# snayfach/MIDAS

Measured on AMD Instinct MI355X. Metric: genomic sites/sec pileup+allele-count, higher is better.
Workload: dtype u8/u32 integer tallies (fp64 only in the two keep_read ratio tests)

## Files before the change

midas_amd/csrc/device_common.h:

```cpp
#pragma once
#include "kernels.h"

namespace midas {
namespace dev {

enum : uint32_t { OP_M = 0, OP_I = 1, OP_D = 2, OP_N = 3, OP_S = 4, OP_H = 5, OP_P = 6, OP_EQ = 7, OP_X = 8 };

enum : uint32_t {
  E_NO_SEQ = 1,
  E_NO_NM = 2,
  E_ZERO_ALIGN = 3,
  E_NO_QUAL = 4,
  E_CIGAR_OVERRUN = 5,
};

typedef uint32_t u32x4_a8 __attribute__((ext_vector_type(4), aligned(8)));
typedef uint32_t u32x4_a4 __attribute__((ext_vector_type(4), aligned(4)));
typedef uint32_t u32x4_a1 __attribute__((ext_vector_type(4), aligned(1)));

__device__ __forceinline__ bool consumes_both(uint32_t op) { return op == OP_M || op == OP_EQ || op == OP_X; }

__device__ __forceinline__ int rec_pos(const uint4& r) { return (int)r.x; }
__device__ __forceinline__ uint32_t rec_off8(const uint4& r) { return r.y; }
__device__ __forceinline__ int rec_l(const uint4& r) { return (int)(r.z & 0x7FFu); }
__device__ __forceinline__ int seg_read_l(const uint4& r) { return (int)((r.z >> 16) & 0x3FFu); }
__device__ __forceinline__ int seg_align_len(const uint4& r) { return (int)((((r.z >> 26) & 0xFu) << 6) | ((r.w >> 10) & 0x3Fu)); }
__device__ __forceinline__ int seg_nm(const uint4& r) { return (int)(r.w & 0x3FFu); }
__device__ __forceinline__ bool seg_first(const uint4& r) { return ((r.z >> 30) & 1u) != 0u; }
__device__ __forceinline__ int rec_qmean(const uint4& r) { return (int)(((r.z >> 11) & 31u) | ((r.w >> 23) & 0xE0u)); }
__device__ __forceinline__ int rec_n(const uint4& r) { return (int)(r.z >> 16); }
__device__ __forceinline__ uint32_t rec_nm(const uint4& r) { return r.w & 0xFFFFu; }
__device__ __forceinline__ int rec_mapq(const uint4& r) { return (int)((r.w >> 16) & 0xFFu); }
__device__ __forceinline__ uint32_t rec_flags(const uint4& r) { return r.w >> 24; }


}
}
```

midas_amd/csrc/pileup_direct.hip:

```cpp
#include "direct_common.h"
#include "pileup_common.h"

#include <type_traits>

namespace midas {

using namespace dev;
using namespace pile;
using namespace direct;

namespace {

#ifdef MIDAS_ISA_MARKS
#define MIDAS_MARK(name) asm volatile("; MARK " name)
#else
#define MIDAS_MARK(name) do { } while (0)
#endif

__device__ __forceinline__ void lds_barrier() { asm volatile("s_waitcnt lgkmcnt(0)\n\ts_barrier" ::: "memory"); }

template <int OFF, int NB>
__device__ __forceinline__ void tally_group(uint32_t b0, uint32_t b1, uint32_t thr, uint32_t abase, uint32_t one) {
  static_assert(NB == 8 || NB == 6, "a group holds 8 bases, or 6 at the end of a 30-base lane");
  const uint32_t c0 = (b0 << 2) & 0x0C0C0C0Cu, c1 = (b1 << 2) & 0x0C0C0C0Cu;
  uint32_t t0, t1, t2, t3, t4, t5, t6, t7;
  unsigned long long m0, m1, m2, m3, m4, m5, m6, m7, save;
  if (NB == 8) {
    asm volatile(
        "v_or_b32_sdwa %[t0], %[ab], %[c0] dst_sel:DWORD dst_unused:UNUSED_PAD src0_sel:DWORD src1_sel:BYTE_0\n\t"
        "v_or_b32_sdwa %[t1], %[ab], %[c0] dst_sel:DWORD dst_unused:UNUSED_PAD src0_sel:DWORD src1_sel:BYTE_1\n\t"
        "v_or_b32_sdwa %[t2], %[ab], %[c0] dst_sel:DWORD dst_unused:UNUSED_PAD src0_sel:DWORD src1_sel:BYTE_2\n\t"
        "v_or_b32_sdwa %[t3], %[ab], %[c0] dst_sel:DWORD dst_unused:UNUSED_PAD src0_sel:DWORD src1_sel:BYTE_3\n\t"
        "v_or_b32_sdwa %[t4], %[ab], %[c1] dst_sel:DWORD dst_unused:UNUSED_PAD src0_sel:DWORD src1_sel:BYTE_0\n\t"
        "v_or_b32_sdwa %[t5], %[ab], %[c1] dst_sel:DWORD dst_unused:UNUSED_PAD src0_sel:DWORD src1_sel:BYTE_1\n\t"
        "v_or_b32_sdwa %[t6], %[ab], %[c1] dst_sel:DWORD dst_unused:UNUSED_PAD src0_sel:DWORD src1_sel:BYTE_2\n\t"
        "v_or_b32_sdwa %[t7], %[ab], %[c1] dst_sel:DWORD dst_unused:UNUSED_PAD src0_sel:DWORD src1_sel:BYTE_3\n\t"
        "v_cmp_ge_u32_sdwa %[m0], %[b0], %[th] src0_sel:BYTE_0 src1_sel:DWORD\n\t"
        "v_cmp_ge_u32_sdwa %[m1], %[b0], %[th] src0_sel:BYTE_1 src1_sel:DWORD\n\t"
        "v_cmp_ge_u32_sdwa %[m2], %[b0], %[th] src0_sel:BYTE_2 src1_sel:DWORD\n\t"
        "v_cmp_ge_u32_sdwa %[m3], %[b0], %[th] src0_sel:BYTE_3 src1_sel:DWORD\n\t"
        "v_cmp_ge_u32_sdwa %[m4], %[b1], %[th] src0_sel:BYTE_0 src1_sel:DWORD\n\t"
        "v_cmp_ge_u32_sdwa %[m5], %[b1], %[th] src0_sel:BYTE_1 src1_sel:DWORD\n\t"
        "v_cmp_ge_u32_sdwa %[m6], %[b1], %[th] src0_sel:BYTE_2 src1_sel:DWORD\n\t"
        "v_cmp_ge_u32_sdwa %[m7], %[b1], %[th] src0_sel:BYTE_3 src1_sel:DWORD\n\t"
        "s_mov_b64 %[sv], exec\n\t"
        "s_mov_b64 exec, %[m0]\n\t"
        "ds_add_u32 %[t0], %[one] offset:%[off]\n\t"
        "s_mov_b64 exec, %[m1]\n\t"
        "ds_add_u32 %[t1], %[one] offset:%[off]+16\n\t"
        "s_mov_b64 exec, %[m2]\n\t"
        "ds_add_u32 %[t2], %[one] offset:%[off]+32\n\t"
        "s_mov_b64 exec, %[m3]\n\t"
        "ds_add_u32 %[t3], %[one] offset:%[off]+48\n\t"
        "s_mov_b64 exec, %[m4]\n\t"
        "ds_add_u32 %[t4], %[one] offset:%[off]+64\n\t"
        "s_mov_b64 exec, %[m5]\n\t"
        "ds_add_u32 %[t5], %[one] offset:%[off]+80\n\t"
        "s_mov_b64 exec, %[m6]\n\t"
        "ds_add_u32 %[t6], %[one] offset:%[off]+96\n\t"
        "s_mov_b64 exec, %[m7]\n\t"
        "ds_add_u32 %[t7], %[one] offset:%[off]+112\n\t"
        "s_mov_b64 exec, %[sv]"
        : [t0] "=&v"(t0), [t1] "=&v"(t1), [t2] "=&v"(t2), [t3] "=&v"(t3), [t4] "=&v"(t4), [t5] "=&v"(t5), [t6] "=&v"(t6),
          [t7] "=&v"(t7), [m0] "=&s"(m0), [m1] "=&s"(m1), [m2] "=&s"(m2), [m3] "=&s"(m3), [m4] "=&s"(m4), [m5] "=&s"(m5),
          [m6] "=&s"(m6), [m7] "=&s"(m7), [sv] "=&s"(save)
        : [b0] "v"(b0), [b1] "v"(b1), [th] "v"(thr), [c0] "v"(c0), [c1] "v"(c1), [ab] "v"(abase), [one] "v"(one), [off] "n"(OFF)
        : "memory");
  } else {
    asm volatile(
        "v_or_b32_sdwa %[t0], %[ab], %[c0] dst_sel:DWORD dst_unused:UNUSED_PAD src0_sel:DWORD src1_sel:BYTE_0\n\t"
        "v_or_b32_sdwa %[t1], %[ab], %[c0] dst_sel:DWORD dst_unused:UNUSED_PAD src0_sel:DWORD src1_sel:BYTE_1\n\t"
        "v_or_b32_sdwa %[t2], %[ab], %[c0] dst_sel:DWORD dst_unused:UNUSED_PAD src0_sel:DWORD src1_sel:BYTE_2\n\t"
        "v_or_b32_sdwa %[t3], %[ab], %[c0] dst_sel:DWORD dst_unused:UNUSED_PAD src0_sel:DWORD src1_sel:BYTE_3\n\t"
        "v_or_b32_sdwa %[t4], %[ab], %[c1] dst_sel:DWORD dst_unused:UNUSED_PAD src0_sel:DWORD src1_sel:BYTE_0\n\t"
        "v_or_b32_sdwa %[t5], %[ab], %[c1] dst_sel:DWORD dst_unused:UNUSED_PAD src0_sel:DWORD src1_sel:BYTE_1\n\t"
        "v_cmp_ge_u32_sdwa %[m0], %[b0], %[th] src0_sel:BYTE_0 src1_sel:DWORD\n\t"
        "v_cmp_ge_u32_sdwa %[m1], %[b0], %[th] src0_sel:BYTE_1 src1_sel:DWORD\n\t"
        "v_cmp_ge_u32_sdwa %[m2], %[b0], %[th] src0_sel:BYTE_2 src1_sel:DWORD\n\t"
        "v_cmp_ge_u32_sdwa %[m3], %[b0], %[th] src0_sel:BYTE_3 src1_sel:DWORD\n\t"
        "v_cmp_ge_u32_sdwa %[m4], %[b1], %[th] src0_sel:BYTE_0 src1_sel:DWORD\n\t"
        "v_cmp_ge_u32_sdwa %[m5], %[b1], %[th] src0_sel:BYTE_1 src1_sel:DWORD\n\t"
        "s_mov_b64 %[sv], exec\n\t"
        "s_mov_b64 exec, %[m0]\n\t"
        "ds_add_u32 %[t0], %[one] offset:%[off]\n\t"
        "s_mov_b64 exec, %[m1]\n\t"
        "ds_add_u32 %[t1], %[one] offset:%[off]+16\n\t"
        "s_mov_b64 exec, %[m2]\n\t"
        "ds_add_u32 %[t2], %[one] offset:%[off]+32\n\t"
        "s_mov_b64 exec, %[m3]\n\t"
        "ds_add_u32 %[t3], %[one] offset:%[off]+48\n\t"
        "s_mov_b64 exec, %[m4]\n\t"
        "ds_add_u32 %[t4], %[one] offset:%[off]+64\n\t"
        "s_mov_b64 exec, %[m5]\n\t"
        "ds_add_u32 %[t5], %[one] offset:%[off]+80\n\t"
        "s_mov_b64 exec, %[sv]"
        : [t0] "=&v"(t0), [t1] "=&v"(t1), [t2] "=&v"(t2), [t3] "=&v"(t3), [t4] "=&v"(t4), [t5] "=&v"(t5), [m0] "=&s"(m0),
          [m1] "=&s"(m1), [m2] "=&s"(m2), [m3] "=&s"(m3), [m4] "=&s"(m4), [m5] "=&s"(m5), [sv] "=&s"(save)
        : [b0] "v"(b0), [b1] "v"(b1), [th] "v"(thr), [c0] "v"(c0), [c1] "v"(c1), [ab] "v"(abase), [one] "v"(one), [off] "n"(OFF)
        : "memory");
  }
}

struct Stream { int rb, n0, total; };

#ifndef MIDAS_DIRECT_BLOCK
#define MIDAS_DIRECT_BLOCK 256
#endif
constexpr int kDirectBlock = MIDAS_DIRECT_BLOCK;
static_assert(kDirectBlock % 64 == 0 && kDirectBlock >= 128 && kDirectBlock <= 1024, "whole wavefronts");
constexpr int kDirectWavesPerSimd = (kWorkgroupsPerCU * kDirectBlock / 64 + 3) / 4;


template <int LB, bool BQ0, int OV = kDirectOverhang>
__global__ __launch_bounds__(kDirectBlock, kDirectWavesPerSimd) void pileup_direct_kernel(DirectParams p) {
  constexpr int TILE = kTileSites;
  constexpr int NWAVES = kDirectBlock / 64;
  constexpr int OUT_IT = (TILE + kDirectBlock - 1) / kDirectBlock;
  static_assert(OV <= TILE, "the overhang is moved by the write-out's first rounds");
  __shared__ __attribute__((aligned(16))) uint32_t lds[4 * (TILE + OV)];
  __shared__ __attribute__((aligned(16))) uint32_t s_kb[33 * 8];
  __shared__ unsigned long long s_stats[MIDAS_STATS];
  __shared__ uint32_t s_next_ticket;
  using table_t = typename std::conditional<(OV > kDirectOverhang), int16_t, int32_t>::type;
  extern __shared__ __attribute__((aligned(16))) uint8_t s_tables_raw[];
  table_t* const s_tables = reinterpret_cast<table_t*>(s_tables_raw);

  const int tid = threadIdx.x;
  const int lane = tid & 63;
  const int wave = __builtin_amdgcn_readfirstlane(tid >> 6);
  const int K = p.chunk_tiles > 1 ? p.chunk_tiles : 1;
  const int T4 = K > 1 ? p.n_chunked_tiles : 0;
  const int n4 = T4 / K;
  const int w_end = n4 + (p.n_tiles - T4);
  auto item_first = [&](int i) -> int { return i < n4 ? i * K : T4 + (i - n4); };
  auto item_end = [&](int i) -> int { return i < n4 ? i * K + K : T4 + (i - n4) + 1; };
#ifdef MIDAS_DIRECT_STATIC
  const bool dynamic = false;
#else
  const bool dynamic = (gridDim.x % kSchedGroups) == 0;
#endif
  const int sched_group = (int)(blockIdx.x % kSchedGroups);
  uint32_t* const sched = p.sched;
  if ((int)blockIdx.x >= w_end) return;
  int c_first = item_first((int)blockIdx.x), c_end = item_end((int)blockIdx.x);
  int i_next = (int)blockIdx.x + (int)gridDim.x;
  i_next = i_next < w_end ? i_next : w_end;
#if MIDAS_SNPS_DEBUG_BITS & 256
  unsigned long long pr_cols = 0, pr_bases = 0, pr_work = 0, pr_sync = 0, pr_out = 0, pr_iters = 0;
  const unsigned long long pr_t0 = __builtin_readcyclecounter();
#define PROBE_NOW() __builtin_readcyclecounter()
#else
#define PROBE_NOW() 0ull
#endif

  {
    uint4* z = reinterpret_cast<uint4*>(lds);
    for (int i = tid; i < TILE + OV; i += kDirectBlock) z[i] = make_uint4(0u, 0u, 0u, 0u);
    for (int i = tid; i < p.table_len; i += kDirectBlock) {
      s_tables[i] = (table_t)p.filt->min_match[i];
      s_tables[p.table_len + i] = (table_t)p.filt->min_align[i];
    }
    for (int i = tid; i < 33 * 8; i += kDirectBlock) {
      const int h = i >> 3, wd = i & 7;
      uint32_t kb = 0;
      for (int k = 0; k < 4; ++k)
        if (4 * wd + k < h) kb |= 0xFFu << (8 * k);
      s_kb[i] = kb;
    }
    if (tid < MIDAS_STATS) s_stats[tid] = 0ull;
  }

  const int lpr = p.lanes_per_read;
  const int rpw = p.reads_per_wave;
  const int g = lane / lpr;
  const int c = lane - g * lpr;
  const int q0 = c * LB;
  const uint32_t lds_base = (uint32_t)(size_t)(__attribute__((address_space(3))) void*)lds;
  const uint32_t thr = BQ0 ? dense_threshold(0) : dense_threshold(p.baseq);
  const int rq = p.readq < 0 ? 0 : (p.readq > 256 ? 256 : p.readq);
  const uint32_t one = 1u;

  const ConstWords c_tiles = (ConstWords)(size_t)p.tiles;
  const ConstWords c_tb = (ConstWords)(size_t)p.tbegin;
  const ConstWords c_te = (ConstWords)(size_t)p.tend;
  auto load_stream = [&](int tt, bool cin) -> Stream {
    Stream s;
    const uint32_t b = cin ? c_te[tt - 1] : c_tb[tt], e = c_te[tt];
    s.rb = e > b ? (int)b : 0;
    s.n0 = e > b ? (int)(e - b) : 0;
    s.total = (s.n0 + rpw - 1) / rpw;
    return s;
  };
  auto reads_in = [&](const Stream& st, int it) -> int {
    const long long left = (long long)st.n0 - (long long)it * rpw;
    return left <= 0 ? 0 : (left < rpw ? (int)left : rpw);
  };

  auto tally_range = [&](bool go, int lo, int hi, int loc0, const uint32_t (&bv)[8], auto sparse_tag) {
    constexpr bool SPARSE = decltype(sparse_tag)::value;
    const uint32_t abase = ((uint32_t)loc0 << 4) + lds_base;
    const bool masked = !(kDebug & 32) && __ballot(go && (lo > 0 || hi < LB)) != 0ull;
    unsigned long long gmask[4];
    if (SPARSE) {
#pragma unroll
      for (int S = 0; S < 4; ++S) gmask[S] = __ballot(go && lo < 8 * S + 8 && hi > 8 * S);
    }
    if (!go) return;
    auto group = [&](auto sidx, auto off, auto nbases) {
      constexpr int S = decltype(sidx)::value;
      if (SPARSE && gmask[S] == 0ull) return;
      uint32_t x0 = bv[2 * S], x1 = bv[2 * S + 1];
      if (masked) {
        const uint2 kh = *reinterpret_cast<const uint2*>(s_kb + 8 * (hi > 32 ? 32 : hi) + 2 * S);
        const uint2 kl = *reinterpret_cast<const uint2*>(s_kb + 8 * (lo < 0 ? 0 : lo) + 2 * S);
        x0 &= kh.x & ~kl.x;
        x1 &= kh.y & ~kl.y;
      }
      tally_group<decltype(off)::value, decltype(nbases)::value>(x0, x1, thr, abase, one);
    };
    using std::integral_constant;
    group(integral_constant<int, 0>{}, integral_constant<int, 0>{}, integral_constant<int, 8>{});
    group(integral_constant<int, 1>{}, integral_constant<int, 128>{}, integral_constant<int, 8>{});
    group(integral_constant<int, 2>{}, integral_constant<int, 256>{}, integral_constant<int, 8>{});
    group(integral_constant<int, 3>{}, integral_constant<int, 384>{}, integral_constant<int, (LB == 32 ? 8 : 6)>{});
  };

  struct Raw { uint32_t pos, l_nc, nmq, off; };
  const uint4* const recs = reinterpret_cast<const uint4*>(p.rec);
  auto fetch = [&](const Stream& st, int it) -> Raw {
    const uint32_t v = (uint32_t)(it * rpw) + (uint32_t)g;
    const uint32_t r = v < (uint32_t)st.n0 ? (uint32_t)st.rb + v : 0u;
    const uint4 x = recs[r];
    Raw f;
    f.pos = x.x; f.l_nc = x.y; f.nmq = x.z; f.off = x.w;
    return f;
  };
  struct Rd { uint32_t pos, nmq, l_nc; };
  struct Dat { uint32_t b[8]; uint32_t cg[4]; uint32_t qs; };
  auto settle = [&](const Raw& f, int n_reads_it, Rd& r, Dat& d) {
    const bool act = g < n_reads_it;
    const uint32_t l_nc = act ? f.l_nc : 0u;
    r.pos = f.pos;
    r.l_nc = l_nc;
    r.nmq = act ? f.nmq : ((uint32_t)kGenIdle << 24);
    const uint32_t off0 = (uint32_t)__builtin_amdgcn_readfirstlane((int)f.off);
    const uint8_t* const base = p.payload + ((unsigned long long)off0 << 3);
    const uint32_t l = l_nc & 0xFFFFu, nc4 = (l_nc >> 16) << 2;
    const uint32_t rel = (f.off - off0) << 3;
    const bool has = (uint32_t)q0 < l && !(kDebug & 128);
    const uint32_t vc = act && !(kDebug & 128) ? rel : 0u;
    const uint32_t vq = act && !(kDebug & 128) ? rel + nc4 : 0u;
    const uint32_t vb = has ? rel + nc4 + 4u + (uint32_t)q0 : 0u;
    const u32x4_a1 ba = *reinterpret_cast<const u32x4_a1*>(base + (size_t)vb);
    const u32x4_a1 bb = *reinterpret_cast<const u32x4_a1*>(base + (size_t)vb + 16);
    const u32x4_a4 cv = *reinterpret_cast<const u32x4_a4*>(base + (size_t)vc);
    const uint32_t qs = *reinterpret_cast<const uint32_t*>(base + (size_t)vq);
    d.b[0] = ba.x; d.b[1] = ba.y; d.b[2] = ba.z; d.b[3] = ba.w;
    d.b[4] = bb.x; d.b[5] = bb.y; d.b[6] = bb.z; d.b[7] = bb.w;
    d.cg[0] = cv.x; d.cg[1] = cv.y; d.cg[2] = cv.z; d.cg[3] = cv.w;
    d.qs = qs;
  };

  Tile tile = load_tile(c_tiles, c_first);
  Stream st = load_stream(c_first, false);
  Raw rawX;
  int nrX = 0;
  Rd rdA, rdB;
  Dat datA, datB;
  auto prime = [&](const Stream& s0) {
    const Raw r0 = fetch(s0, wave);
    rawX = fetch(s0, wave + NWAVES);
    nrX = reads_in(s0, wave + NWAVES);
    settle(r0, reads_in(s0, wave), rdA, datA);
  };
  prime(st);
  __syncthreads();

  uint32_t acc_cov = 0u;
  unsigned long long acc_depth = 0ull;
  int t = c_first;
  for (;;) {
    const int tile_len = tile.len;
    const int tile_start = tile.start;
    const bool in_chunk = t + 1 < c_end;
    const bool more = in_chunk || i_next < w_end;
    const int wn = in_chunk ? t + 1 : (more ? item_first(i_next) : t);
    const bool carry = in_chunk && (!p.chunk_ok || p.chunk_ok[c_first / K] != 0);
    const bool cout = carry && (int32_t)c_tiles[8 * (size_t)wn] == tile.contig;
    const int next_len = (int32_t)c_tiles[8 * (size_t)wn + 2];
    const int ext_len = tile_len + (cout ? (next_len < OV ? next_len : OV) : 0);
    const int it_hi = st.total;
    uint32_t w_aligned = 0, w_mapped = 0;
    constexpr int REF_IT = (TILE + 4 * kDirectBlock - 1) / (4 * kDirectBlock);

    const int n_w = it_hi > wave ? (it_hi - wave + NWAVES - 1) / NWAVES : 0;
    const bool xt = more && n_w >= 2;
    Stream xs = st;
    if (xt) xs = load_stream(wn, cout);
    auto iteration = [&](int it, int k_it, Rd& rd_cur, Dat& dat_cur, Rd& rd_n, Dat& dat_n) {
      const unsigned long long pt0 = PROBE_NOW();
      MIDAS_MARK("settle");
      settle(rawX, nrX, rd_n, dat_n);
      {
        const int kf = k_it + 2;
        const bool over = xt && kf >= n_w;
        Stream fs;
        fs.rb = over ? xs.rb : st.rb; fs.n0 = over ? xs.n0 : st.n0; fs.total = over ? xs.total : st.total;
        const int fi = wave + (over ? kf - n_w : kf) * NWAVES;
        rawX = fetch(fs, fi);
        nrX = reads_in(fs, fi);
      }
#if MIDAS_SNPS_DEBUG_BITS & 256
      asm volatile("" :: "v"(rd_n.pos), "v"(rd_n.l_nc));
      const unsigned long long pt1 = PROBE_NOW();
      asm volatile("" :: "v"(dat_cur.b[0]), "v"(dat_cur.b[7]), "v"(dat_cur.qs), "v"(dat_cur.cg[3]));
      const unsigned long long pt2 = PROBE_NOW();
      pr_cols += pt1 - pt0; pr_bases += pt2 - pt1; pr_iters += 1;
#endif

      if (kDebug & 4) {
        asm volatile("" :: "v"(dat_cur.b[0]), "v"(dat_cur.b[7]), "v"(dat_cur.qs), "v"(dat_cur.cg[0]), "v"(rd_cur.pos));
        return;
      }
      MIDAS_MARK("qsum");
      const int pos = (int)rd_cur.pos;
      const int l = (int)(rd_cur.l_nc & 0xFFFFu);
      const uint32_t nc = rd_cur.l_nc >> 16;
      const int nb = l - q0 < LB ? (l - q0 < 0 ? 0 : l - q0) : LB;
      const bool has = nb > 0;
      uint32_t qsum = (kDebug & (64 | 512)) ? 0x00FFFFFFu : dat_cur.qs;
      const bool t_noqual = (qsum & kDenseQualAbsent) != 0u;
      qsum &= ~kDenseQualAbsent;
      const uint32_t nm16 = rd_cur.nmq & 0xFFFFu;
      const int nm = (int)nm16, mapq = (int)((rd_cur.nmq >> 16) & 0xFFu);
      const bool act = !((rd_cur.nmq >> 24) & kGenIdle);

      MIDAS_MARK("shape");
      ReadShape sh;
      sh.lead = 0u; sh.m1 = (uint32_t)l; sh.ins = 0u; sh.del = 0u; sh.alen = (uint32_t)l;
      bool shaped = nc == 1u && op_is_match(dat_cur.cg[0] & 15u) && (dat_cur.cg[0] >> 4) == (uint32_t)l && l >= 1;
      if (kDebug & 512) shaped = true;
      if (__ballot(act && !shaped) != 0ull) {
        ReadShape s2;
        const bool ok = decode_shape(dat_cur.cg[0], dat_cur.cg[1], dat_cur.cg[2], dat_cur.cg[3], nc, (uint32_t)l, &s2);
        if (!shaped) { sh = s2; shaped = ok; }
      }
      const bool fast = act && shaped && nm16 != 0xFFFFu && pos >= 0 && pos < tile.contig_len;
      const bool slow = act && !fast;

      MIDAS_MARK("filter");
      const int lead = (int)sh.lead, align_len = (int)sh.alen;
      bool keep, owner;
      uint32_t err;
      {
        const int min_match = (kDebug & 512) ? 0 : s_tables[align_len < p.table_len ? align_len : 0];
        const int min_align = (kDebug & 512) ? 0 : s_tables[p.table_len + (l < p.table_len ? l : 0)];
        const bool t_pid = align_len - nm < min_match;
        const bool t_drop = ((int)qsum < rq * l) | (mapq < p.mapq_min) | (align_len < min_align);
        err = (fast && !t_pid && t_noqual) ? (uint32_t)E_NO_QUAL : 0u;
        keep = fast && !(t_pid | t_noqual | t_drop);
        const int rel = pos - tile_start;
        owner = fast && rel >= 0 && rel < tile_len;
        const int qa1 = lead + (int)sh.m1, qb0 = qa1 + (int)sh.ins, qb1 = lead + align_len;
        const int loc_a = rel + (q0 - lead);
        const int loc_b = loc_a + (int)sh.del - (int)sh.ins;
        int lo_a = lead - q0, hi_a = qa1 - q0, lo_b = qb0 - q0, hi_b = qb1 - q0;
        lo_a = lo_a > -loc_a ? lo_a : -loc_a;
        lo_a = lo_a > 0 ? lo_a : 0;
        hi_a = hi_a < ext_len - loc_a ? hi_a : ext_len - loc_a;
        hi_a = hi_a < nb ? hi_a : nb;
        lo_b = lo_b > -loc_b ? lo_b : -loc_b;
        lo_b = lo_b > 0 ? lo_b : 0;
        hi_b = hi_b < ext_len - loc_b ? hi_b : ext_len - loc_b;
        hi_b = hi_b < nb ? hi_b : nb;
        const bool go_a = keep && lo_a < hi_a, go_b = keep && lo_b < hi_b;
        const bool go1 = go_a | go_b;
        MIDAS_MARK("pass1");
        if (!(kDebug & 1) && __ballot(go1) != 0ull)
          tally_range(go1, go_a ? lo_a : lo_b, go_a ? hi_a : hi_b, go_a ? loc_a : loc_b, dat_cur.b, std::false_type{});
        const bool go2 = go_a & go_b;
        MIDAS_MARK("pass2");
        if (!(kDebug & (1 | 16)) && __ballot(go2) != 0ull) tally_range(go2, lo_b, hi_b, loc_b, dat_cur.b, std::true_type{});
      }
      MIDAS_MARK("slowgate");
      if (__ballot(slow) != 0ull) {
        const uint32_t idx = (uint32_t)(st.rb + it * rpw + g);
        CigarView cg;
        cg.c0 = dat_cur.cg[0]; cg.c1 = dat_cur.cg[1]; cg.c2 = dat_cur.cg[2]; cg.c3 = dat_cur.cg[3];
        cg.p = reinterpret_cast<const uint32_t*>(p.payload);
        if (slow && nc > 4u) cg.p = reinterpret_cast<const uint32_t*>(p.payload + ((unsigned long long)p.rec[idx].off8 << 3));
        const uint32_t ncs = slow ? nc : 0u;
        long long qs = 0, qe = 0;
        query_bounds(cg, ncs, l, &qs, &qe);
        long long al = qe - qs;
        al = al < 0 ? 0 : (al > 2047 ? 2047 : al);
        const int align_g = (int)al;
        bool t_over = false;
        {
          long long qpos = 0, rpos = pos;
          const long long clen = tile.contig_len;
          for_each_op(cg, ncs, [&](uint32_t, uint32_t v) {
            const uint32_t op = v & 15u;
            const long long len = (long long)(v >> 4);
            if (op_is_match(op)) {
              if (qpos + len > (long long)l) {
                const long long qs2 = qpos > (long long)l ? qpos : (long long)l;
                const long long rs = rpos + (qs2 - qpos), re = rpos + len;
                if (rs < clen && re > 0) t_over = true;
              }
              qpos += len;
              rpos += len;
            } else if (op == OP_I || op == OP_S || (op == OP_P && p.pad_advances)) {
              qpos += len;
            } else if (op == OP_D || op == OP_N) {
              rpos += len;
            }
            return true;
          });
        }
        const int min_match = s_tables[align_g < p.table_len ? align_g : 0];
        const int min_align = s_tables[p.table_len + (l < p.table_len ? l : 0)];
        const bool t_noseq = l == 0;
        const bool t_nonm = nm16 == 0xFFFFu;
        const bool t_zero = align_g == 0;
        const bool t_pid = align_g - nm < min_match;
        const bool t_drop = ((int)qsum < rq * l) | (mapq < p.mapq_min) | (align_g < min_align);
        uint32_t e = t_over ? (uint32_t)E_CIGAR_OVERRUN : 0u;
        e = t_drop ? 0u : e;
        e = t_noqual ? (uint32_t)E_NO_QUAL : e;
        e = t_pid ? 0u : e;
        e = t_zero ? (uint32_t)E_ZERO_ALIGN : e;
        e = t_nonm ? (uint32_t)E_NO_NM : e;
        e = t_noseq ? (uint32_t)E_NO_SEQ : e;
        const bool keep_s = slow && !(t_noseq | t_nonm | t_zero | t_pid | t_noqual | t_drop | t_over);
        int cpos = pos < 0 ? 0 : pos;
        cpos = cpos > tile.contig_len - 1 ? tile.contig_len - 1 : cpos;
        const bool owner_s = slow && cpos >= tile_start && cpos < tile_start + tile_len && !(tile.halo && pos < 0);
        if (slow) { err = e; keep = keep_s; owner = owner_s; }
        const int rel = pos - tile_start;
        int rrel = (rel > (1 << 25) || rel < -(1 << 30)) ? (1 << 25) : rel;
        uint32_t k = 0;
        int qpos = 0, jlo = 0, jhi = 0, loc0 = 0;
        const int q1 = q0 + nb;
        auto next_segment = [&]() -> bool {
          while (k < nc) {
            const uint32_t v = cg[k];
            ++k;
            const uint32_t op = v & 15u;
            const int len = (int)(v >> 4);
            const bool m = consumes_both(op);
            bool found = false;
            if (m) {
              const int lo = qpos > q0 ? qpos : q0;
              const int hi = (qpos + len) < q1 ? (qpos + len) : q1;
              found = lo < hi;
              if (found) { jlo = lo - q0; jhi = hi - q0; loc0 = rrel + (q0 - qpos); }
            }
            if (m || op == OP_I || op == OP_S || (op == OP_P && p.pad_advances)) { qpos += len; qpos = qpos > (1 << 29) ? (1 << 29) : qpos; }
            if (m || op == OP_D || op == OP_N) { rrel += len; rrel = rrel > (1 << 29) ? (1 << 29) : rrel; }
            if (found) return true;
          }
          return false;
        };
        bool walking = keep_s && has;
        if (walking) walking = next_segment();
        while (__ballot(walking) != 0ull) {
          const int lo = jlo > -loc0 ? jlo : -loc0;
          const int hi = jhi < ext_len - loc0 ? jhi : ext_len - loc0;
          if (!(kDebug & 1)) tally_range(walking && lo < hi, lo, hi, loc0, dat_cur.b, std::true_type{});
          walking = (walking && k < nc) ? next_segment() : false;
        }
      }
      MIDAS_MARK("counters");
      const bool head = owner && c == 0;
      w_aligned += (uint32_t)__popcll(__ballot(head));
      w_mapped += (uint32_t)__popcll(__ballot(head && keep));
      const bool walk_err = slow && tile.halo && pos < 0 && c == 0 && err == (uint32_t)E_CIGAR_OVERRUN;
      if ((head && err) || walk_err) {
        const uint32_t idx = (uint32_t)(st.rb + it * rpw + g);
        atomicMin(p.err, ((unsigned long long)idx << 8) | err);
      }

      MIDAS_MARK("iterend");
#if MIDAS_SNPS_DEBUG_BITS & 256
      pr_work += PROBE_NOW() - pt2;
#endif
    };
    {
      int it = wave, k_it = 0;
      bool odd = false;
      while (it < it_hi) {
        iteration(it, k_it, rdA, datA, rdB, datB);
        it += NWAVES;
        ++k_it;
        if (it >= it_hi) { odd = true; break; }
        iteration(it, k_it, rdB, datB, rdA, datA);
        it += NWAVES;
        ++k_it;
      }
      if (odd) { rdA = rdB; datA = datB; }
    }

    uint32_t refw[REF_IT];
    if (p.out_allele) {
      const uint8_t* ref = p.ref + tile.site_base;
#pragma unroll
      for (int it = 0; it < REF_IT; ++it) {
        const int i = 4 * (tid + it * kDirectBlock);
        if (i + 4 <= tile_len) refw[it] = *reinterpret_cast<const u32_a1*>(ref + i);
      }
    }
    if (lane == 0) {
      if (w_aligned) atomicAdd(&s_stats[MIDAS_STAT_ALIGNED], (unsigned long long)w_aligned);
      if (w_mapped) atomicAdd(&s_stats[MIDAS_STAT_MAPPED], (unsigned long long)w_mapped);
    }
    const int tn = wn;
    const Tile ntile = load_tile(c_tiles, tn);
    const Stream nst = load_stream(tn, cout);
    const bool take = more && !in_chunk;
    const unsigned long long ps0 = PROBE_NOW();
    if (more && !xt) {
      const Raw r0 = fetch(nst, wave);
      rawX = fetch(nst, wave + NWAVES);
      nrX = reads_in(nst, wave + NWAVES);
      lds_barrier();
      settle(r0, reads_in(nst, wave), rdA, datA);
    } else {
      lds_barrier();
    }
    const unsigned long long ps1 = PROBE_NOW();
    uint32_t ticket = 0;
    if (dynamic && take && tid == 0) ticket = atomicAdd(&sched[32 * sched_group], 1u);

    {
      uint4* out = reinterpret_cast<uint4*>(p.out_counts) + ((kDebug & 8) ? 0 : tile.site_base);
      uint4* lds4 = reinterpret_cast<uint4*>(lds);
      const int lim = (kDebug & 2) ? 0 : tile_len;
#pragma unroll
      for (int it = 0; it < OUT_IT; ++it) {
        const int i = tid + it * kDirectBlock;
        if (i < lim) {
          const uint4 v = lds4[i];
          if (cout && i < OV) {
            lds4[i] = lds4[TILE + i];
            lds4[TILE + i] = make_uint4(0u, 0u, 0u, 0u);
          } else {
            lds4[i] = make_uint4(0u, 0u, 0u, 0u);
          }
          u32x4_a8 nv; nv.x = v.x; nv.y = v.y; nv.z = v.z; nv.w = v.w;
          __builtin_nontemporal_store(nv, reinterpret_cast<u32x4_a8*>(out + i));
          const uint32_t d = v.x + v.y + v.z + v.w;
          acc_cov += d > 0u ? 1u : 0u;
          acc_depth += d;
        }
      }
    }
    if (p.out_allele && !(kDebug & 2)) {
      const uint8_t* ref = p.ref + tile.site_base;
      uint8_t* al = p.out_allele + tile.site_base;
#pragma unroll
      for (int it = 0; it < REF_IT; ++it) {
        const int i = 4 * (tid + it * kDirectBlock);
        if (i + 4 <= tile_len) {
          __builtin_nontemporal_store(upper4(refw[it]), reinterpret_cast<u32_a1*>(al + i));
        } else {
          for (int j = i; j < tile_len; ++j) {
            uint32_t ch = ref[j];
            if (ch >= 'a' && ch <= 'z') ch -= 32u;
            al[j] = (uint8_t)ch;
          }
        }
      }
    }
    if (dynamic && take && tid == 0) s_next_ticket = ticket;
    lds_barrier();
#if MIDAS_SNPS_DEBUG_BITS & 256
    pr_sync += ps1 - ps0;
    pr_out += PROBE_NOW() - ps1;
#else
    (void)ps0; (void)ps1;
#endif
    if (take) {
      const long long nn = dynamic ? 2ll * (long long)gridDim.x + (long long)kSchedGroups * s_next_ticket + sched_group
                                   : (long long)i_next + (long long)gridDim.x;
      c_first = item_first(i_next);
      c_end = item_end(i_next);
      i_next = __builtin_amdgcn_readfirstlane((int)(nn < (long long)w_end ? nn : (long long)w_end));
    }
    const bool flush = !more || ntile.species != tile.species;
    if (flush) {
      for (int d = 32; d >= 1; d >>= 1) {
        acc_cov += __shfl_down(acc_cov, d);
        acc_depth += __shfl_down(acc_depth, d);
      }
      if (lane == 0) {
        if (acc_cov) atomicAdd(&s_stats[MIDAS_STAT_COVERED], (unsigned long long)acc_cov);
        if (acc_depth) atomicAdd(&s_stats[MIDAS_STAT_DEPTH], acc_depth);
      }
      acc_cov = 0u;
      acc_depth = 0ull;
      lds_barrier();
      if (tid < MIDAS_STATS) {
        const unsigned long long v = s_stats[tid];
        if (v) atomicAdd(&p.stats[(size_t)tile.species * MIDAS_STATS + tid], v);
        s_stats[tid] = 0ull;
      }
      if (!more) {
        if (dynamic && tid == 0) {
          if (atomicAdd(&sched[32 * kSchedGroups], 1u) == gridDim.x - 1u) {
            for (int k = 0; k <= kSchedGroups; ++k) sched[32 * k] = 0u;
          }
        }
        break;
      }
      lds_barrier();
    }
    t = tn;
    tile = ntile;
    st = nst;
  }
#if MIDAS_SNPS_DEBUG_BITS & 256
  if (lane == 0 && p.probe) {
    unsigned long long* o = p.probe + ((size_t)blockIdx.x * NWAVES + wave) * 8;
    uint32_t hw_id, xcc_id;
    asm volatile("s_getreg_b32 %0, hwreg(HW_REG_HW_ID)\n\ts_getreg_b32 %1, hwreg(HW_REG_XCC_ID)" : "=s"(hw_id), "=s"(xcc_id));
    o[0] = pr_cols; o[1] = (unsigned long long)hw_id | ((unsigned long long)xcc_id << 32); o[2] = pr_work; o[3] = pr_sync; o[4] = pr_out; o[5] = pr_iters;
    o[6] = __builtin_readcyclecounter() - pr_t0; o[7] = 0ull;
  }
#endif
#undef PROBE_NOW
}

}

int direct_lane_bases(int32_t max_l_seq) {
  const int l = max_l_seq > 0 ? max_l_seq : 1;
  return (l + 31) / 32 < (l + 29) / 30 ? 32 : 30;
}

hipError_t launch_pileup_direct(const DirectParams& p, int lane_bases, hipStream_t stream) {
  if (p.n_tiles <= 0) return hipSuccess;
  const size_t dyn_lds = (size_t)p.table_len * 2 * (p.overhang > kDirectOverhang ? sizeof(int16_t) : sizeof(int32_t));
  const int k = p.chunk_tiles > 1 ? p.chunk_tiles : 1;
  const int n_items = k > 1 ? p.n_chunked_tiles / k + (p.n_tiles - p.n_chunked_tiles) : p.n_tiles;
  const int grid = n_items < p.grid_blocks ? n_items : p.grid_blocks;
  const bool bq0 = p.baseq <= 0;
  if (p.overhang > kDirectOverhang) {
    if (lane_bases == 32) {
      if (bq0) hipLaunchKernelGGL((pileup_direct_kernel<32, true, kDirectOverhangLong>), dim3(grid), dim3(kDirectBlock), dyn_lds, stream, p);
      else hipLaunchKernelGGL((pileup_direct_kernel<32, false, kDirectOverhangLong>), dim3(grid), dim3(kDirectBlock), dyn_lds, stream, p);
    } else {
      if (bq0) hipLaunchKernelGGL((pileup_direct_kernel<30, true, kDirectOverhangLong>), dim3(grid), dim3(kDirectBlock), dyn_lds, stream, p);
      else hipLaunchKernelGGL((pileup_direct_kernel<30, false, kDirectOverhangLong>), dim3(grid), dim3(kDirectBlock), dyn_lds, stream, p);
    }
  } else if (lane_bases == 32) {
    if (bq0) hipLaunchKernelGGL((pileup_direct_kernel<32, true>), dim3(grid), dim3(kDirectBlock), dyn_lds, stream, p);
    else hipLaunchKernelGGL((pileup_direct_kernel<32, false>), dim3(grid), dim3(kDirectBlock), dyn_lds, stream, p);
  } else {
    if (bq0) hipLaunchKernelGGL((pileup_direct_kernel<30, true>), dim3(grid), dim3(kDirectBlock), dyn_lds, stream, p);
    else hipLaunchKernelGGL((pileup_direct_kernel<30, false>), dim3(grid), dim3(kDirectBlock), dyn_lds, stream, p);
  }
  return hipGetLastError();
}

}
```

Measured before the change: 96.86 billion.

## Add 38-base lane variant to cut lanes per read for mid-length reads

Generalises the direct pileup kernel to a variable number of base words per lane and adds a 38-base-per-lane instantiation, chosen when reads are over 96 bases and 38-base lanes need fewer lanes per read than 32. Fewer lanes per read lets each wave hold more reads per iteration, which is meant to raise throughput. The cost is an extra 8-byte load, a fifth tally group per lane and more registers, which may reduce occupancy. An attic variant file that precomputes the masked rows ahead of the tally is also added, but it is not built.

Result: faster. 100.9 billion, median of 6 (+4.1%).

```diff
diff --git a/attic/variants/pileup_direct_rows_ahead.hip b/attic/variants/pileup_direct_rows_ahead.hip
--- /dev/null
+++ b/attic/variants/pileup_direct_rows_ahead.hip
@@ -0,0 +1,707 @@
+#include "direct_common.h"
+#include "pileup_common.h"
+
+#include <type_traits>
+
+namespace midas {
+
+using namespace dev;
+using namespace pile;
+using namespace direct;
+
+namespace {
+
+#ifdef MIDAS_ISA_MARKS
+#define MIDAS_MARK(name) asm volatile("; MARK " name)
+#else
+#define MIDAS_MARK(name) do { } while (0)
+#endif
+
+__device__ __forceinline__ void lds_barrier() { asm volatile("s_waitcnt lgkmcnt(0)\n\ts_barrier" ::: "memory"); }
+
+template <int OFF, int NB>
+__device__ __forceinline__ void tally_group(uint32_t b0, uint32_t b1, uint32_t thr, uint32_t abase, uint32_t one) {
+  static_assert(NB == 8 || NB == 6, "a group holds 8 bases, or 6 at the end of a 30- or 38-base lane");
+  const uint32_t c0 = (b0 << 2) & 0x0C0C0C0Cu, c1 = (b1 << 2) & 0x0C0C0C0Cu;
+  uint32_t t0, t1, t2, t3, t4, t5, t6, t7;
+  unsigned long long m0, m1, m2, m3, m4, m5, m6, m7, save;
+  if (NB == 8) {
+    asm volatile(
+        "v_or_b32_sdwa %[t0], %[ab], %[c0] dst_sel:DWORD dst_unused:UNUSED_PAD src0_sel:DWORD src1_sel:BYTE_0\n\t"
+        "v_or_b32_sdwa %[t1], %[ab], %[c0] dst_sel:DWORD dst_unused:UNUSED_PAD src0_sel:DWORD src1_sel:BYTE_1\n\t"
+        "v_or_b32_sdwa %[t2], %[ab], %[c0] dst_sel:DWORD dst_unused:UNUSED_PAD src0_sel:DWORD src1_sel:BYTE_2\n\t"
+        "v_or_b32_sdwa %[t3], %[ab], %[c0] dst_sel:DWORD dst_unused:UNUSED_PAD src0_sel:DWORD src1_sel:BYTE_3\n\t"
+        "v_or_b32_sdwa %[t4], %[ab], %[c1] dst_sel:DWORD dst_unused:UNUSED_PAD src0_sel:DWORD src1_sel:BYTE_0\n\t"
+        "v_or_b32_sdwa %[t5], %[ab], %[c1] dst_sel:DWORD dst_unused:UNUSED_PAD src0_sel:DWORD src1_sel:BYTE_1\n\t"
+        "v_or_b32_sdwa %[t6], %[ab], %[c1] dst_sel:DWORD dst_unused:UNUSED_PAD src0_sel:DWORD src1_sel:BYTE_2\n\t"
+        "v_or_b32_sdwa %[t7], %[ab], %[c1] dst_sel:DWORD dst_unused:UNUSED_PAD src0_sel:DWORD src1_sel:BYTE_3\n\t"
+        "v_cmp_ge_u32_sdwa %[m0], %[b0], %[th] src0_sel:BYTE_0 src1_sel:DWORD\n\t"
+        "v_cmp_ge_u32_sdwa %[m1], %[b0], %[th] src0_sel:BYTE_1 src1_sel:DWORD\n\t"
+        "v_cmp_ge_u32_sdwa %[m2], %[b0], %[th] src0_sel:BYTE_2 src1_sel:DWORD\n\t"
+        "v_cmp_ge_u32_sdwa %[m3], %[b0], %[th] src0_sel:BYTE_3 src1_sel:DWORD\n\t"
+        "v_cmp_ge_u32_sdwa %[m4], %[b1], %[th] src0_sel:BYTE_0 src1_sel:DWORD\n\t"
+        "v_cmp_ge_u32_sdwa %[m5], %[b1], %[th] src0_sel:BYTE_1 src1_sel:DWORD\n\t"
+        "v_cmp_ge_u32_sdwa %[m6], %[b1], %[th] src0_sel:BYTE_2 src1_sel:DWORD\n\t"
+        "v_cmp_ge_u32_sdwa %[m7], %[b1], %[th] src0_sel:BYTE_3 src1_sel:DWORD\n\t"
+        "s_mov_b64 %[sv], exec\n\t"
+        "s_mov_b64 exec, %[m0]\n\t"
+        "ds_add_u32 %[t0], %[one] offset:%[off]\n\t"
+        "s_mov_b64 exec, %[m1]\n\t"
+        "ds_add_u32 %[t1], %[one] offset:%[off]+16\n\t"
+        "s_mov_b64 exec, %[m2]\n\t"
+        "ds_add_u32 %[t2], %[one] offset:%[off]+32\n\t"
+        "s_mov_b64 exec, %[m3]\n\t"
+        "ds_add_u32 %[t3], %[one] offset:%[off]+48\n\t"
+        "s_mov_b64 exec, %[m4]\n\t"
+        "ds_add_u32 %[t4], %[one] offset:%[off]+64\n\t"
+        "s_mov_b64 exec, %[m5]\n\t"
+        "ds_add_u32 %[t5], %[one] offset:%[off]+80\n\t"
+        "s_mov_b64 exec, %[m6]\n\t"
+        "ds_add_u32 %[t6], %[one] offset:%[off]+96\n\t"
+        "s_mov_b64 exec, %[m7]\n\t"
+        "ds_add_u32 %[t7], %[one] offset:%[off]+112\n\t"
+        "s_mov_b64 exec, %[sv]"
+        : [t0] "=&v"(t0), [t1] "=&v"(t1), [t2] "=&v"(t2), [t3] "=&v"(t3), [t4] "=&v"(t4), [t5] "=&v"(t5), [t6] "=&v"(t6),
+          [t7] "=&v"(t7), [m0] "=&s"(m0), [m1] "=&s"(m1), [m2] "=&s"(m2), [m3] "=&s"(m3), [m4] "=&s"(m4), [m5] "=&s"(m5),
+          [m6] "=&s"(m6), [m7] "=&s"(m7), [sv] "=&s"(save)
+        : [b0] "v"(b0), [b1] "v"(b1), [th] "v"(thr), [c0] "v"(c0), [c1] "v"(c1), [ab] "v"(abase), [one] "v"(one), [off] "n"(OFF)
+        : "memory");
+  } else {
+    asm volatile(
+        "v_or_b32_sdwa %[t0], %[ab], %[c0] dst_sel:DWORD dst_unused:UNUSED_PAD src0_sel:DWORD src1_sel:BYTE_0\n\t"
+        "v_or_b32_sdwa %[t1], %[ab], %[c0] dst_sel:DWORD dst_unused:UNUSED_PAD src0_sel:DWORD src1_sel:BYTE_1\n\t"
+        "v_or_b32_sdwa %[t2], %[ab], %[c0] dst_sel:DWORD dst_unused:UNUSED_PAD src0_sel:DWORD src1_sel:BYTE_2\n\t"
+        "v_or_b32_sdwa %[t3], %[ab], %[c0] dst_sel:DWORD dst_unused:UNUSED_PAD src0_sel:DWORD src1_sel:BYTE_3\n\t"
+        "v_or_b32_sdwa %[t4], %[ab], %[c1] dst_sel:DWORD dst_unused:UNUSED_PAD src0_sel:DWORD src1_sel:BYTE_0\n\t"
+        "v_or_b32_sdwa %[t5], %[ab], %[c1] dst_sel:DWORD dst_unused:UNUSED_PAD src0_sel:DWORD src1_sel:BYTE_1\n\t"
+        "v_cmp_ge_u32_sdwa %[m0], %[b0], %[th] src0_sel:BYTE_0 src1_sel:DWORD\n\t"
+        "v_cmp_ge_u32_sdwa %[m1], %[b0], %[th] src0_sel:BYTE_1 src1_sel:DWORD\n\t"
+        "v_cmp_ge_u32_sdwa %[m2], %[b0], %[th] src0_sel:BYTE_2 src1_sel:DWORD\n\t"
+        "v_cmp_ge_u32_sdwa %[m3], %[b0], %[th] src0_sel:BYTE_3 src1_sel:DWORD\n\t"
+        "v_cmp_ge_u32_sdwa %[m4], %[b1], %[th] src0_sel:BYTE_0 src1_sel:DWORD\n\t"
+        "v_cmp_ge_u32_sdwa %[m5], %[b1], %[th] src0_sel:BYTE_1 src1_sel:DWORD\n\t"
+        "s_mov_b64 %[sv], exec\n\t"
+        "s_mov_b64 exec, %[m0]\n\t"
+        "ds_add_u32 %[t0], %[one] offset:%[off]\n\t"
+        "s_mov_b64 exec, %[m1]\n\t"
+        "ds_add_u32 %[t1], %[one] offset:%[off]+16\n\t"
+        "s_mov_b64 exec, %[m2]\n\t"
+        "ds_add_u32 %[t2], %[one] offset:%[off]+32\n\t"
+        "s_mov_b64 exec, %[m3]\n\t"
+        "ds_add_u32 %[t3], %[one] offset:%[off]+48\n\t"
+        "s_mov_b64 exec, %[m4]\n\t"
+        "ds_add_u32 %[t4], %[one] offset:%[off]+64\n\t"
+        "s_mov_b64 exec, %[m5]\n\t"
+        "ds_add_u32 %[t5], %[one] offset:%[off]+80\n\t"
+        "s_mov_b64 exec, %[sv]"
+        : [t0] "=&v"(t0), [t1] "=&v"(t1), [t2] "=&v"(t2), [t3] "=&v"(t3), [t4] "=&v"(t4), [t5] "=&v"(t5), [m0] "=&s"(m0),
+          [m1] "=&s"(m1), [m2] "=&s"(m2), [m3] "=&s"(m3), [m4] "=&s"(m4), [m5] "=&s"(m5), [sv] "=&s"(save)
+        : [b0] "v"(b0), [b1] "v"(b1), [th] "v"(thr), [c0] "v"(c0), [c1] "v"(c1), [ab] "v"(abase), [one] "v"(one), [off] "n"(OFF)
+        : "memory");
+  }
+}
+
+struct Stream { int rb, n0, total; };
+
+#ifndef MIDAS_DIRECT_BLOCK
+#define MIDAS_DIRECT_BLOCK 256
+#endif
+constexpr int kDirectBlock = MIDAS_DIRECT_BLOCK;
+static_assert(kDirectBlock % 64 == 0 && kDirectBlock >= 128 && kDirectBlock <= 1024, "whole wavefronts");
+#ifndef MIDAS_DIRECT_ROWS_AHEAD
+#define MIDAS_DIRECT_ROWS_AHEAD 1
+#endif
+constexpr int kDirectWavesPerSimd = (kWorkgroupsPerCU * kDirectBlock / 64 + 3) / 4;
+
+
+template <int LB, bool BQ0, int OV = kDirectOverhang>
+__global__ __launch_bounds__(kDirectBlock, kDirectWavesPerSimd) void pileup_direct_kernel(DirectParams p) {
+  static_assert(LB == 30 || LB == 32 || LB == 38, "a lane's bases: 8 or 10 words of four base bytes");
+  constexpr int TILE = kTileSites;
+  constexpr int NW = (LB + 3) / 4;
+  constexpr int NG = (LB + 7) / 8;
+  constexpr int KROWS = (LB > 32 ? LB : 32) + 1;
+  constexpr int NWAVES = kDirectBlock / 64;
+  constexpr int OUT_IT = (TILE + kDirectBlock - 1) / kDirectBlock;
+  static_assert(OV <= TILE, "the overhang is moved by the write-out's first rounds");
+  __shared__ __attribute__((aligned(16))) uint32_t lds[4 * (TILE + OV)];
+  __shared__ __attribute__((aligned(16))) uint32_t s_kb[KROWS * NW];
+  __shared__ unsigned long long s_stats[MIDAS_STATS];
+  __shared__ uint32_t s_next_ticket;
+  using table_t = typename std::conditional<(OV > kDirectOverhang), int16_t, int32_t>::type;
+  extern __shared__ __attribute__((aligned(16))) uint8_t s_tables_raw[];
+  table_t* const s_tables = reinterpret_cast<table_t*>(s_tables_raw);
+
+  const int tid = threadIdx.x;
+  const int lane = tid & 63;
+  const int wave = __builtin_amdgcn_readfirstlane(tid >> 6);
+  const int K = p.chunk_tiles > 1 ? p.chunk_tiles : 1;
+  const int T4 = K > 1 ? p.n_chunked_tiles : 0;
+  const int n4 = T4 / K;
+  const int w_end = n4 + (p.n_tiles - T4);
+  auto item_first = [&](int i) -> int { return i < n4 ? i * K : T4 + (i - n4); };
+  auto item_end = [&](int i) -> int { return i < n4 ? i * K + K : T4 + (i - n4) + 1; };
+#ifdef MIDAS_DIRECT_STATIC
+  const bool dynamic = false;
+#else
+  const bool dynamic = (gridDim.x % kSchedGroups) == 0;
+#endif
+  const int sched_group = (int)(blockIdx.x % kSchedGroups);
+  uint32_t* const sched = p.sched;
+  if ((int)blockIdx.x >= w_end) return;
+  int c_first = item_first((int)blockIdx.x), c_end = item_end((int)blockIdx.x);
+  int i_next = (int)blockIdx.x + (int)gridDim.x;
+  i_next = i_next < w_end ? i_next : w_end;
+#if MIDAS_SNPS_DEBUG_BITS & 256
+  unsigned long long pr_cols = 0, pr_bases = 0, pr_work = 0, pr_sync = 0, pr_out = 0, pr_iters = 0;
+  const unsigned long long pr_t0 = __builtin_readcyclecounter();
+#define PROBE_NOW() __builtin_readcyclecounter()
+#else
+#define PROBE_NOW() 0ull
+#endif
+
+  {
+    uint4* z = reinterpret_cast<uint4*>(lds);
+    for (int i = tid; i < TILE + OV; i += kDirectBlock) z[i] = make_uint4(0u, 0u, 0u, 0u);
+    for (int i = tid; i < p.table_len; i += kDirectBlock) {
+      s_tables[i] = (table_t)p.filt->min_match[i];
+      s_tables[p.table_len + i] = (table_t)p.filt->min_align[i];
+    }
+    for (int i = tid; i < KROWS * NW; i += kDirectBlock) {
+      const int h = i / NW, wd = i - h * NW;
+      uint32_t kb = 0;
+      for (int k = 0; k < 4; ++k)
+        if (4 * wd + k < h) kb |= 0xFFu << (8 * k);
+      s_kb[i] = kb;
+    }
+    if (tid < MIDAS_STATS) s_stats[tid] = 0ull;
+  }
+
+  const int lpr = p.lanes_per_read;
+  const int rpw = p.reads_per_wave;
+  const int g = lane / lpr;
+  const int c = lane - g * lpr;
+  const int q0 = c * LB;
+  const uint32_t lds_base = (uint32_t)(size_t)(__attribute__((address_space(3))) void*)lds;
+  const uint32_t thr = BQ0 ? dense_threshold(0) : dense_threshold(p.baseq);
+  const int rq = p.readq < 0 ? 0 : (p.readq > 256 ? 256 : p.readq);
+  const uint32_t one = 1u;
+
+  const ConstWords c_tiles = (ConstWords)(size_t)p.tiles;
+  const ConstWords c_tb = (ConstWords)(size_t)p.tbegin;
+  const ConstWords c_te = (ConstWords)(size_t)p.tend;
+  auto load_stream = [&](int tt, bool cin) -> Stream {
+    Stream s;
+    const uint32_t b = cin ? c_te[tt - 1] : c_tb[tt], e = c_te[tt];
+    s.rb = e > b ? (int)b : 0;
+    s.n0 = e > b ? (int)(e - b) : 0;
+    s.total = (s.n0 + rpw - 1) / rpw;
+    return s;
+  };
+  auto reads_in = [&](const Stream& st, int it) -> int {
+    const long long left = (long long)st.n0 - (long long)it * rpw;
+    return left <= 0 ? 0 : (left < rpw ? (int)left : rpw);
+  };
+
+  auto tally_range = [&](bool go, int lo, int hi, int loc0, const uint32_t (&bv)[NW], auto sparse_tag) {
+    constexpr bool SPARSE = decltype(sparse_tag)::value;
+    const uint32_t abase = ((uint32_t)loc0 << 4) + lds_base;
+    const bool masked = !(kDebug & 32) && __ballot(go && (lo > 0 || hi < LB)) != 0ull;
+    unsigned long long gmask[NG];
+    if (SPARSE) {
+#pragma unroll
+      for (int S = 0; S < NG; ++S) gmask[S] = __ballot(go && lo < 8 * S + 8 && hi > 8 * S);
+    }
+    if (!go) return;
+    const uint32_t* const row_hi = s_kb + NW * (hi > KROWS - 1 ? KROWS - 1 : hi);
+    const uint32_t* const row_lo = s_kb + NW * (lo < 0 ? 0 : lo);
+#if MIDAS_DIRECT_ROWS_AHEAD
+    uint32_t xv[NW];
+#pragma unroll
+    for (int w = 0; w < NW; ++w) xv[w] = bv[w];
+    if (masked) {
+#pragma unroll
+      for (int S = 0; S < NG; ++S) {
+        if (SPARSE && gmask[S] == 0ull) continue;
+        const uint2 kh = *reinterpret_cast<const uint2*>(row_hi + 2 * S);
+        const uint2 kl = *reinterpret_cast<const uint2*>(row_lo + 2 * S);
+        xv[2 * S] &= kh.x & ~kl.x;
+        xv[2 * S + 1] &= kh.y & ~kl.y;
+      }
+    }
+#endif
+    auto group = [&](auto sidx, auto nbases) {
+      constexpr int S = decltype(sidx)::value;
+      if (SPARSE && gmask[S] == 0ull) return;
+#if MIDAS_DIRECT_ROWS_AHEAD
+      const uint32_t x0 = xv[2 * S], x1 = xv[2 * S + 1];
+#else
+      uint32_t x0 = bv[2 * S], x1 = bv[2 * S + 1];
+      if (masked) {
+        const uint2 kh = *reinterpret_cast<const uint2*>(row_hi + 2 * S);
+        const uint2 kl = *reinterpret_cast<const uint2*>(row_lo + 2 * S);
+        x0 &= kh.x & ~kl.x;
+        x1 &= kh.y & ~kl.y;
+      }
+#endif
+      tally_group<128 * S, decltype(nbases)::value>(x0, x1, thr, abase, one);
+    };
+    using std::integral_constant;
+    group(integral_constant<int, 0>{}, integral_constant<int, 8>{});
+    group(integral_constant<int, 1>{}, integral_constant<int, 8>{});
+    group(integral_constant<int, 2>{}, integral_constant<int, 8>{});
+    group(integral_constant<int, 3>{}, integral_constant<int, (NG > 4 ? 8 : LB - 24)>{});
+    if constexpr (NG > 4) group(integral_constant<int, 4>{}, integral_constant<int, LB - 32>{});
+  };
+
+  struct Raw { uint32_t pos, l_nc, nmq, off; };
+  const uint4* const recs = reinterpret_cast<const uint4*>(p.rec);
+  auto fetch = [&](const Stream& st, int it) -> Raw {
+    const uint32_t v = (uint32_t)(it * rpw) + (uint32_t)g;
+    const uint32_t r = v < (uint32_t)st.n0 ? (uint32_t)st.rb + v : 0u;
+    const uint4 x = recs[r];
+    Raw f;
+    f.pos = x.x; f.l_nc = x.y; f.nmq = x.z; f.off = x.w;
+    return f;
+  };
+  struct Rd { uint32_t pos, nmq, l_nc; };
+  struct Dat { uint32_t b[NW]; uint32_t cg[4]; uint32_t qs; };
+  auto settle = [&](const Raw& f, int n_reads_it, Rd& r, Dat& d) {
+    const bool act = g < n_reads_it;
+    const uint32_t l_nc = act ? f.l_nc : 0u;
+    r.pos = f.pos;
+    r.l_nc = l_nc;
+    r.nmq = act ? f.nmq : ((uint32_t)kGenIdle << 24);
+    const uint32_t off0 = (uint32_t)__builtin_amdgcn_readfirstlane((int)f.off);
+    const uint8_t* const base = p.payload + ((unsigned long long)off0 << 3);
+    const uint32_t l = l_nc & 0xFFFFu, nc4 = (l_nc >> 16) << 2;
+    const uint32_t rel = (f.off - off0) << 3;
+    const bool has = (uint32_t)q0 < l && !(kDebug & 128);
+    const uint32_t vc = act && !(kDebug & 128) ? rel : 0u;
+    const uint32_t vq = act && !(kDebug & 128) ? rel + nc4 : 0u;
+    const uint32_t vb = has ? rel + nc4 + 4u + (uint32_t)q0 : 0u;
+    const u32x4_a1 ba = *reinterpret_cast<const u32x4_a1*>(base + (size_t)vb);
+    const u32x4_a1 bb = *reinterpret_cast<const u32x4_a1*>(base + (size_t)vb + 16);
+    const u32x4_a4 cv = *reinterpret_cast<const u32x4_a4*>(base + (size_t)vc);
+    const uint32_t qs = *reinterpret_cast<const uint32_t*>(base + (size_t)vq);
+    d.b[0] = ba.x; d.b[1] = ba.y; d.b[2] = ba.z; d.b[3] = ba.w;
+    d.b[4] = bb.x; d.b[5] = bb.y; d.b[6] = bb.z; d.b[7] = bb.w;
+    if constexpr (NW > 8) {
+      const u32x2_a1 bc = *reinterpret_cast<const u32x2_a1*>(base + (size_t)vb + 32);
+      d.b[8] = bc.x; d.b[9] = bc.y;
+    }
+    d.cg[0] = cv.x; d.cg[1] = cv.y; d.cg[2] = cv.z; d.cg[3] = cv.w;
+    d.qs = qs;
+  };
+
+  Tile tile = load_tile(c_tiles, c_first);
+  Stream st = load_stream(c_first, false);
+  Raw rawX;
+  int nrX = 0;
+  Rd rdA, rdB;
+  Dat datA, datB;
+  auto prime = [&](const Stream& s0) {
+    const Raw r0 = fetch(s0, wave);
+    rawX = fetch(s0, wave + NWAVES);
+    nrX = reads_in(s0, wave + NWAVES);
+    settle(r0, reads_in(s0, wave), rdA, datA);
+  };
+  prime(st);
+  __syncthreads();
+
+  uint32_t acc_cov = 0u;
+  unsigned long long acc_depth = 0ull;
+  int t = c_first;
+  for (;;) {
+    const int tile_len = tile.len;
+    const int tile_start = tile.start;
+    const bool in_chunk = t + 1 < c_end;
+    const bool more = in_chunk || i_next < w_end;
+    const int wn = in_chunk ? t + 1 : (more ? item_first(i_next) : t);
+    const bool carry = in_chunk && (!p.chunk_ok || p.chunk_ok[c_first / K] != 0);
+    const bool cout = carry && (int32_t)c_tiles[8 * (size_t)wn] == tile.contig;
+    const int next_len = (int32_t)c_tiles[8 * (size_t)wn + 2];
+    const int ext_len = tile_len + (cout ? (next_len < OV ? next_len : OV) : 0);
+    const int it_hi = st.total;
+    uint32_t w_aligned = 0, w_mapped = 0;
+    constexpr int REF_IT = (TILE + 4 * kDirectBlock - 1) / (4 * kDirectBlock);
+
+    const int n_w = it_hi > wave ? (it_hi - wave + NWAVES - 1) / NWAVES : 0;
+    const bool xt = more && n_w >= 2;
+    Stream xs = st;
+    if (xt) xs = load_stream(wn, cout);
+    auto iteration = [&](int it, int k_it, Rd& rd_cur, Dat& dat_cur, Rd& rd_n, Dat& dat_n) {
+      const unsigned long long pt0 = PROBE_NOW();
+      MIDAS_MARK("settle");
+      settle(rawX, nrX, rd_n, dat_n);
+      {
+        const int kf = k_it + 2;
+        const bool over = xt && kf >= n_w;
+        Stream fs;
+        fs.rb = over ? xs.rb : st.rb; fs.n0 = over ? xs.n0 : st.n0; fs.total = over ? xs.total : st.total;
+        const int fi = wave + (over ? kf - n_w : kf) * NWAVES;
+        rawX = fetch(fs, fi);
+        nrX = reads_in(fs, fi);
+      }
+#if MIDAS_SNPS_DEBUG_BITS & 256
+      asm volatile("" :: "v"(rd_n.pos), "v"(rd_n.l_nc));
+      const unsigned long long pt1 = PROBE_NOW();
+      asm volatile("" :: "v"(dat_cur.b[0]), "v"(dat_cur.b[NW - 1]), "v"(dat_cur.qs), "v"(dat_cur.cg[3]));
+      const unsigned long long pt2 = PROBE_NOW();
+      pr_cols += pt1 - pt0; pr_bases += pt2 - pt1; pr_iters += 1;
+#endif
+
+      if (kDebug & 4) {
+        asm volatile("" :: "v"(dat_cur.b[0]), "v"(dat_cur.b[NW - 1]), "v"(dat_cur.qs), "v"(dat_cur.cg[0]), "v"(rd_cur.pos));
+        return;
+      }
+      MIDAS_MARK("qsum");
+      const int pos = (int)rd_cur.pos;
+      const int l = (int)(rd_cur.l_nc & 0xFFFFu);
+      const uint32_t nc = rd_cur.l_nc >> 16;
+      const int nb = l - q0 < LB ? (l - q0 < 0 ? 0 : l - q0) : LB;
+      const bool has = nb > 0;
+      uint32_t qsum = (kDebug & (64 | 512)) ? 0x00FFFFFFu : dat_cur.qs;
+      const bool t_noqual = (qsum & kDenseQualAbsent) != 0u;
+      qsum &= ~kDenseQualAbsent;
+      const uint32_t nm16 = rd_cur.nmq & 0xFFFFu;
+      const int nm = (int)nm16, mapq = (int)((rd_cur.nmq >> 16) & 0xFFu);
+      const bool act = !((rd_cur.nmq >> 24) & kGenIdle);
+
+      MIDAS_MARK("shape");
+      ReadShape sh;
+      sh.lead = 0u; sh.m1 = (uint32_t)l; sh.ins = 0u; sh.del = 0u; sh.alen = (uint32_t)l;
+      bool shaped = nc == 1u && op_is_match(dat_cur.cg[0] & 15u) && (dat_cur.cg[0] >> 4) == (uint32_t)l && l >= 1;
+      if (kDebug & 512) shaped = true;
+      if (__ballot(act && !shaped) != 0ull) {
+        ReadShape s2;
+        const bool ok = decode_shape(dat_cur.cg[0], dat_cur.cg[1], dat_cur.cg[2], dat_cur.cg[3], nc, (uint32_t)l, &s2);
+        if (!shaped) { sh = s2; shaped = ok; }
+      }
+      const bool fast = act && shaped && nm16 != 0xFFFFu && pos >= 0 && pos < tile.contig_len;
+      const bool slow = act && !fast;
+
+      MIDAS_MARK("filter");
+      const int lead = (int)sh.lead, align_len = (int)sh.alen;
+      bool keep, owner;
+      uint32_t err;
+      {
+        const int min_match = (kDebug & 512) ? 0 : s_tables[align_len < p.table_len ? align_len : 0];
+        const int min_align = (kDebug & 512) ? 0 : s_tables[p.table_len + (l < p.table_len ? l : 0)];
+        const bool t_pid = align_len - nm < min_match;
+        const bool t_drop = ((int)qsum < rq * l) | (mapq < p.mapq_min) | (align_len < min_align);
+        err = (fast && !t_pid && t_noqual) ? (uint32_t)E_NO_QUAL : 0u;
+        keep = fast && !(t_pid | t_noqual | t_drop);
+        const int rel = pos - tile_start;
+        owner = fast && rel >= 0 && rel < tile_len;
+        const int qa1 = lead + (int)sh.m1, qb0 = qa1 + (int)sh.ins, qb1 = lead + align_len;
+        const int loc_a = rel + (q0 - lead);
+        const int loc_b = loc_a + (int)sh.del - (int)sh.ins;
+        int lo_a = lead - q0, hi_a = qa1 - q0, lo_b = qb0 - q0, hi_b = qb1 - q0;
+        lo_a = lo_a > -loc_a ? lo_a : -loc_a;
+        lo_a = lo_a > 0 ? lo_a : 0;
+        hi_a = hi_a < ext_len - loc_a ? hi_a : ext_len - loc_a;
+        hi_a = hi_a < nb ? hi_a : nb;
+        lo_b = lo_b > -loc_b ? lo_b : -loc_b;
+        lo_b = lo_b > 0 ? lo_b : 0;
+        hi_b = hi_b < ext_len - loc_b ? hi_b : ext_len - loc_b;
+        hi_b = hi_b < nb ? hi_b : nb;
+        const bool go_a = keep && lo_a < hi_a, go_b = keep && lo_b < hi_b;
+        const bool go1 = go_a | go_b;
+        MIDAS_MARK("pass1");
+        if (!(kDebug & 1) && __ballot(go1) != 0ull)
+          tally_range(go1, go_a ? lo_a : lo_b, go_a ? hi_a : hi_b, go_a ? loc_a : loc_b, dat_cur.b, std::false_type{});
+        const bool go2 = go_a & go_b;
+        MIDAS_MARK("pass2");
+        if (!(kDebug & (1 | 16)) && __ballot(go2) != 0ull) tally_range(go2, lo_b, hi_b, loc_b, dat_cur.b, std::true_type{});
+      }
+      MIDAS_MARK("slowgate");
+      if (__ballot(slow) != 0ull) {
+        const uint32_t idx = (uint32_t)(st.rb + it * rpw + g);
+        CigarView cg;
+        cg.c0 = dat_cur.cg[0]; cg.c1 = dat_cur.cg[1]; cg.c2 = dat_cur.cg[2]; cg.c3 = dat_cur.cg[3];
+        cg.p = reinterpret_cast<const uint32_t*>(p.payload);
+        if (slow && nc > 4u) cg.p = reinterpret_cast<const uint32_t*>(p.payload + ((unsigned long long)p.rec[idx].off8 << 3));
+        const uint32_t ncs = slow ? nc : 0u;
+        long long qs = 0, qe = 0;
+        query_bounds(cg, ncs, l, &qs, &qe);
+        long long al = qe - qs;
+        al = al < 0 ? 0 : (al > 2047 ? 2047 : al);
+        const int align_g = (int)al;
+        bool t_over = false;
+        {
+          long long qpos = 0, rpos = pos;
+          const long long clen = tile.contig_len;
+          for_each_op(cg, ncs, [&](uint32_t, uint32_t v) {
+            const uint32_t op = v & 15u;
+            const long long len = (long long)(v >> 4);
+            if (op_is_match(op)) {
+              if (qpos + len > (long long)l) {
+                const long long qs2 = qpos > (long long)l ? qpos : (long long)l;
+                const long long rs = rpos + (qs2 - qpos), re = rpos + len;
+                if (rs < clen && re > 0) t_over = true;
+              }
+              qpos += len;
+              rpos += len;
+            } else if (op == OP_I || op == OP_S || (op == OP_P && p.pad_advances)) {
+              qpos += len;
+            } else if (op == OP_D || op == OP_N) {
+              rpos += len;
+            }
+            return true;
+          });
+        }
+        const int min_match = s_tables[align_g < p.table_len ? align_g : 0];
+        const int min_align = s_tables[p.table_len + (l < p.table_len ? l : 0)];
+        const bool t_noseq = l == 0;
+        const bool t_nonm = nm16 == 0xFFFFu;
+        const bool t_zero = align_g == 0;
+        const bool t_pid = align_g - nm < min_match;
+        const bool t_drop = ((int)qsum < rq * l) | (mapq < p.mapq_min) | (align_g < min_align);
+        uint32_t e = t_over ? (uint32_t)E_CIGAR_OVERRUN : 0u;
+        e = t_drop ? 0u : e;
+        e = t_noqual ? (uint32_t)E_NO_QUAL : e;
+        e = t_pid ? 0u : e;
+        e = t_zero ? (uint32_t)E_ZERO_ALIGN : e;
+        e = t_nonm ? (uint32_t)E_NO_NM : e;
+        e = t_noseq ? (uint32_t)E_NO_SEQ : e;
+        const bool keep_s = slow && !(t_noseq | t_nonm | t_zero | t_pid | t_noqual | t_drop | t_over);
+        int cpos = pos < 0 ? 0 : pos;
+        cpos = cpos > tile.contig_len - 1 ? tile.contig_len - 1 : cpos;
+        const bool owner_s = slow && cpos >= tile_start && cpos < tile_start + tile_len && !(tile.halo && pos < 0);
+        if (slow) { err = e; keep = keep_s; owner = owner_s; }
+        const int rel = pos - tile_start;
+        int rrel = (rel > (1 << 25) || rel < -(1 << 30)) ? (1 << 25) : rel;
+        uint32_t k = 0;
+        int qpos = 0, jlo = 0, jhi = 0, loc0 = 0;
+        const int q1 = q0 + nb;
+        auto next_segment = [&]() -> bool {
+          while (k < nc) {
+            const uint32_t v = cg[k];
+            ++k;
+            const uint32_t op = v & 15u;
+            const int len = (int)(v >> 4);
+            const bool m = consumes_both(op);
+            bool found = false;
+            if (m) {
+              const int lo = qpos > q0 ? qpos : q0;
+              const int hi = (qpos + len) < q1 ? (qpos + len) : q1;
+              found = lo < hi;
+              if (found) { jlo = lo - q0; jhi = hi - q0; loc0 = rrel + (q0 - qpos); }
+            }
+            if (m || op == OP_I || op == OP_S || (op == OP_P && p.pad_advances)) { qpos += len; qpos = qpos > (1 << 29) ? (1 << 29) : qpos; }
+            if (m || op == OP_D || op == OP_N) { rrel += len; rrel = rrel > (1 << 29) ? (1 << 29) : rrel; }
+            if (found) return true;
+          }
+          return false;
+        };
+        bool walking = keep_s && has;
+        if (walking) walking = next_segment();
+        while (__ballot(walking) != 0ull) {
+          const int lo = jlo > -loc0 ? jlo : -loc0;
+          const int hi = jhi < ext_len - loc0 ? jhi : ext_len - loc0;
+          if (!(kDebug & 1)) tally_range(walking && lo < hi, lo, hi, loc0, dat_cur.b, std::true_type{});
+          walking = (walking && k < nc) ? next_segment() : false;
+        }
+      }
+      MIDAS_MARK("counters");
+      const bool head = owner && c == 0;
+      w_aligned += (uint32_t)__popcll(__ballot(head));
+      w_mapped += (uint32_t)__popcll(__ballot(head && keep));
+      const bool walk_err = slow && tile.halo && pos < 0 && c == 0 && err == (uint32_t)E_CIGAR_OVERRUN;
+      if ((head && err) || walk_err) {
+        const uint32_t idx = (uint32_t)(st.rb + it * rpw + g);
+        atomicMin(p.err, ((unsigned long long)idx << 8) | err);
+      }
+
+      MIDAS_MARK("iterend");
+#if MIDAS_SNPS_DEBUG_BITS & 256
+      pr_work += PROBE_NOW() - pt2;
+#endif
+    };
+    {
+      int it = wave, k_it = 0;
+      bool odd = false;
+      while (it < it_hi) {
+        iteration(it, k_it, rdA, datA, rdB, datB);
+        it += NWAVES;
+        ++k_it;
+        if (it >= it_hi) { odd = true; break; }
+        iteration(it, k_it, rdB, datB, rdA, datA);
+        it += NWAVES;
+        ++k_it;
+      }
+      if (odd) { rdA = rdB; datA = datB; }
+    }
+
+    uint32_t refw[REF_IT];
+    if (p.out_allele) {
+      const uint8_t* ref = p.ref + tile.site_base;
+#pragma unroll
+      for (int it = 0; it < REF_IT; ++it) {
+        const int i = 4 * (tid + it * kDirectBlock);
+        if (i + 4 <= tile_len) refw[it] = *reinterpret_cast<const u32_a1*>(ref + i);
+      }
+    }
+    if (lane == 0) {
+      if (w_aligned) atomicAdd(&s_stats[MIDAS_STAT_ALIGNED], (unsigned long long)w_aligned);
+      if (w_mapped) atomicAdd(&s_stats[MIDAS_STAT_MAPPED], (unsigned long long)w_mapped);
+    }
+    const int tn = wn;
+    const Tile ntile = load_tile(c_tiles, tn);
+    const Stream nst = load_stream(tn, cout);
+    const bool take = more && !in_chunk;
+    const unsigned long long ps0 = PROBE_NOW();
+    if (more && !xt) {
+      const Raw r0 = fetch(nst, wave);
+      rawX = fetch(nst, wave + NWAVES);
+      nrX = reads_in(nst, wave + NWAVES);
+      lds_barrier();
+      settle(r0, reads_in(nst, wave), rdA, datA);
+    } else {
+      lds_barrier();
+    }
+    const unsigned long long ps1 = PROBE_NOW();
+    uint32_t ticket = 0;
+    if (dynamic && take && tid == 0) ticket = atomicAdd(&sched[32 * sched_group], 1u);
+
+    {
+      uint4* out = reinterpret_cast<uint4*>(p.out_counts) + ((kDebug & 8) ? 0 : tile.site_base);
+      uint4* lds4 = reinterpret_cast<uint4*>(lds);
+      const int lim = (kDebug & 2) ? 0 : tile_len;
+#pragma unroll
+      for (int it = 0; it < OUT_IT; ++it) {
+        const int i = tid + it * kDirectBlock;
+        if (i < lim) {
+          const uint4 v = lds4[i];
+          if (cout && i < OV) {
+            lds4[i] = lds4[TILE + i];
+            lds4[TILE + i] = make_uint4(0u, 0u, 0u, 0u);
+          } else {
+            lds4[i] = make_uint4(0u, 0u, 0u, 0u);
+          }
+          u32x4_a8 nv; nv.x = v.x; nv.y = v.y; nv.z = v.z; nv.w = v.w;
+          __builtin_nontemporal_store(nv, reinterpret_cast<u32x4_a8*>(out + i));
+          const uint32_t d = v.x + v.y + v.z + v.w;
+          acc_cov += d > 0u ? 1u : 0u;
+          acc_depth += d;
+        }
+      }
+    }
+    if (p.out_allele && !(kDebug & 2)) {
+      const uint8_t* ref = p.ref + tile.site_base;
+      uint8_t* al = p.out_allele + tile.site_base;
+#pragma unroll
+      for (int it = 0; it < REF_IT; ++it) {
+        const int i = 4 * (tid + it * kDirectBlock);
+        if (i + 4 <= tile_len) {
+          __builtin_nontemporal_store(upper4(refw[it]), reinterpret_cast<u32_a1*>(al + i));
+        } else {
+          for (int j = i; j < tile_len; ++j) {
+            uint32_t ch = ref[j];
+            if (ch >= 'a' && ch <= 'z') ch -= 32u;
+            al[j] = (uint8_t)ch;
+          }
+        }
+      }
+    }
+    if (dynamic && take && tid == 0) s_next_ticket = ticket;
+    lds_barrier();
+#if MIDAS_SNPS_DEBUG_BITS & 256
+    pr_sync += ps1 - ps0;
+    pr_out += PROBE_NOW() - ps1;
+#else
+    (void)ps0; (void)ps1;
+#endif
+    if (take) {
+      const long long nn = dynamic ? 2ll * (long long)gridDim.x + (long long)kSchedGroups * s_next_ticket + sched_group
+                                   : (long long)i_next + (long long)gridDim.x;
+      c_first = item_first(i_next);
+      c_end = item_end(i_next);
+      i_next = __builtin_amdgcn_readfirstlane((int)(nn < (long long)w_end ? nn : (long long)w_end));
+    }
+    const bool flush = !more || ntile.species != tile.species;
+    if (flush) {
+      for (int d = 32; d >= 1; d >>= 1) {
+        acc_cov += __shfl_down(acc_cov, d);
+        acc_depth += __shfl_down(acc_depth, d);
+      }
+      if (lane == 0) {
+        if (acc_cov) atomicAdd(&s_stats[MIDAS_STAT_COVERED], (unsigned long long)acc_cov);
+        if (acc_depth) atomicAdd(&s_stats[MIDAS_STAT_DEPTH], acc_depth);
+      }
+      acc_cov = 0u;
+      acc_depth = 0ull;
+      lds_barrier();
+      if (tid < MIDAS_STATS) {
+        const unsigned long long v = s_stats[tid];
+        if (v) atomicAdd(&p.stats[(size_t)tile.species * MIDAS_STATS + tid], v);
+        s_stats[tid] = 0ull;
+      }
+      if (!more) {
+        if (dynamic && tid == 0) {
+          if (atomicAdd(&sched[32 * kSchedGroups], 1u) == gridDim.x - 1u) {
+            for (int k = 0; k <= kSchedGroups; ++k) sched[32 * k] = 0u;
+          }
+        }
+        break;
+      }
+      lds_barrier();
+    }
+    t = tn;
+    tile = ntile;
+    st = nst;
+  }
+#if MIDAS_SNPS_DEBUG_BITS & 256
+  if (lane == 0 && p.probe) {
+    unsigned long long* o = p.probe + ((size_t)blockIdx.x * NWAVES + wave) * 8;
+    uint32_t hw_id, xcc_id;
+    asm volatile("s_getreg_b32 %0, hwreg(HW_REG_HW_ID)\n\ts_getreg_b32 %1, hwreg(HW_REG_XCC_ID)" : "=s"(hw_id), "=s"(xcc_id));
+    o[0] = pr_cols; o[1] = (unsigned long long)hw_id | ((unsigned long long)xcc_id << 32); o[2] = pr_work; o[3] = pr_sync; o[4] = pr_out; o[5] = pr_iters;
+    o[6] = __builtin_readcyclecounter() - pr_t0; o[7] = 0ull;
+  }
+#endif
+#undef PROBE_NOW
+}
+
+}
+
+int direct_lane_bases(int32_t max_l_seq) {
+  const int l = max_l_seq > 0 ? max_l_seq : 1;
+  const int best = (l + 31) / 32 < (l + 29) / 30 ? 32 : 30;
+#ifndef MIDAS_DIRECT_NO_LB38
+  if (best == 30 && l > 96 && l <= kDirectOverhang && (l + 37) / 38 < (l + 31) / 32) return 38;
+#endif
+  return best;
+}
+
+hipError_t launch_pileup_direct(const DirectParams& p, int lane_bases, hipStream_t stream) {
+  if (p.n_tiles <= 0) return hipSuccess;
+  const size_t dyn_lds = (size_t)p.table_len * 2 * (p.overhang > kDirectOverhang ? sizeof(int16_t) : sizeof(int32_t));
+  const int k = p.chunk_tiles > 1 ? p.chunk_tiles : 1;
+  const int n_items = k > 1 ? p.n_chunked_tiles / k + (p.n_tiles - p.n_chunked_tiles) : p.n_tiles;
+  const int grid = n_items < p.grid_blocks ? n_items : p.grid_blocks;
+  const bool bq0 = p.baseq <= 0;
+  if (lane_bases != 30 && lane_bases != 32 && !(lane_bases == 38 && p.overhang <= kDirectOverhang)) return hipErrorInvalidValue;
+  if (p.overhang > kDirectOverhang) {
+    if (lane_bases == 32) {
+      if (bq0) hipLaunchKernelGGL((pileup_direct_kernel<32, true, kDirectOverhangLong>), dim3(grid), dim3(kDirectBlock), dyn_lds, stream, p);
+      else hipLaunchKernelGGL((pileup_direct_kernel<32, false, kDirectOverhangLong>), dim3(grid), dim3(kDirectBlock), dyn_lds, stream, p);
+    } else {
+      if (bq0) hipLaunchKernelGGL((pileup_direct_kernel<30, true, kDirectOverhangLong>), dim3(grid), dim3(kDirectBlock), dyn_lds, stream, p);
+      else hipLaunchKernelGGL((pileup_direct_kernel<30, false, kDirectOverhangLong>), dim3(grid), dim3(kDirectBlock), dyn_lds, stream, p);
+    }
+  } else if (lane_bases == 38) {
+    if (bq0) hipLaunchKernelGGL((pileup_direct_kernel<38, true>), dim3(grid), dim3(kDirectBlock), dyn_lds, stream, p);
+    else hipLaunchKernelGGL((pileup_direct_kernel<38, false>), dim3(grid), dim3(kDirectBlock), dyn_lds, stream, p);
+  } else if (lane_bases == 32) {
+    if (bq0) hipLaunchKernelGGL((pileup_direct_kernel<32, true>), dim3(grid), dim3(kDirectBlock), dyn_lds, stream, p);
+    else hipLaunchKernelGGL((pileup_direct_kernel<32, false>), dim3(grid), dim3(kDirectBlock), dyn_lds, stream, p);
+  } else {
+    if (bq0) hipLaunchKernelGGL((pileup_direct_kernel<30, true>), dim3(grid), dim3(kDirectBlock), dyn_lds, stream, p);
+    else hipLaunchKernelGGL((pileup_direct_kernel<30, false>), dim3(grid), dim3(kDirectBlock), dyn_lds, stream, p);
+  }
+  return hipGetLastError();
+}
+
+}
diff --git a/midas_amd/csrc/device_common.h b/midas_amd/csrc/device_common.h
--- a/midas_amd/csrc/device_common.h
+++ b/midas_amd/csrc/device_common.h
@@ -17,6 +17,7 @@
 typedef uint32_t u32x4_a8 __attribute__((ext_vector_type(4), aligned(8)));
 typedef uint32_t u32x4_a4 __attribute__((ext_vector_type(4), aligned(4)));
 typedef uint32_t u32x4_a1 __attribute__((ext_vector_type(4), aligned(1)));
+typedef uint32_t u32x2_a1 __attribute__((ext_vector_type(2), aligned(1)));
 
 __device__ __forceinline__ bool consumes_both(uint32_t op) { return op == OP_M || op == OP_EQ || op == OP_X; }
 
diff --git a/midas_amd/csrc/pileup_direct.hip b/midas_amd/csrc/pileup_direct.hip
--- a/midas_amd/csrc/pileup_direct.hip
+++ b/midas_amd/csrc/pileup_direct.hip
@@ -21,7 +21,7 @@
 
 template <int OFF, int NB>
 __device__ __forceinline__ void tally_group(uint32_t b0, uint32_t b1, uint32_t thr, uint32_t abase, uint32_t one) {
-  static_assert(NB == 8 || NB == 6, "a group holds 8 bases, or 6 at the end of a 30-base lane");
+  static_assert(NB == 8 || NB == 6, "a group holds 8 bases, or 6 at the end of a 30- or 38-base lane");
   const uint32_t c0 = (b0 << 2) & 0x0C0C0C0Cu, c1 = (b1 << 2) & 0x0C0C0C0Cu;
   uint32_t t0, t1, t2, t3, t4, t5, t6, t7;
   unsigned long long m0, m1, m2, m3, m4, m5, m6, m7, save;
@@ -113,12 +113,16 @@
 
 template <int LB, bool BQ0, int OV = kDirectOverhang>
 __global__ __launch_bounds__(kDirectBlock, kDirectWavesPerSimd) void pileup_direct_kernel(DirectParams p) {
+  static_assert(LB == 30 || LB == 32 || LB == 38, "a lane's bases: 8 or 10 words of four base bytes");
   constexpr int TILE = kTileSites;
+  constexpr int NW = (LB + 3) / 4;
+  constexpr int NG = (LB + 7) / 8;
+  constexpr int KROWS = (LB > 32 ? LB : 32) + 1;
   constexpr int NWAVES = kDirectBlock / 64;
   constexpr int OUT_IT = (TILE + kDirectBlock - 1) / kDirectBlock;
   static_assert(OV <= TILE, "the overhang is moved by the write-out's first rounds");
   __shared__ __attribute__((aligned(16))) uint32_t lds[4 * (TILE + OV)];
-  __shared__ __attribute__((aligned(16))) uint32_t s_kb[33 * 8];
+  __shared__ __attribute__((aligned(16))) uint32_t s_kb[KROWS * NW];
   __shared__ unsigned long long s_stats[MIDAS_STATS];
   __shared__ uint32_t s_next_ticket;
   using table_t = typename std::conditional<(OV > kDirectOverhang), int16_t, int32_t>::type;
@@ -160,8 +164,8 @@
       s_tables[i] = (table_t)p.filt->min_match[i];
       s_tables[p.table_len + i] = (table_t)p.filt->min_align[i];
     }
-    for (int i = tid; i < 33 * 8; i += kDirectBlock) {
-      const int h = i >> 3, wd = i & 7;
+    for (int i = tid; i < KROWS * NW; i += kDirectBlock) {
+      const int h = i / NW, wd = i - h * NW;
       uint32_t kb = 0;
       for (int k = 0; k < 4; ++k)
         if (4 * wd + k < h) kb |= 0xFFu << (8 * k);
@@ -196,33 +200,36 @@
     return left <= 0 ? 0 : (left < rpw ? (int)left : rpw);
   };
 
-  auto tally_range = [&](bool go, int lo, int hi, int loc0, const uint32_t (&bv)[8], auto sparse_tag) {
+  auto tally_range = [&](bool go, int lo, int hi, int loc0, const uint32_t (&bv)[NW], auto sparse_tag) {
     constexpr bool SPARSE = decltype(sparse_tag)::value;
     const uint32_t abase = ((uint32_t)loc0 << 4) + lds_base;
     const bool masked = !(kDebug & 32) && __ballot(go && (lo > 0 || hi < LB)) != 0ull;
-    unsigned long long gmask[4];
+    unsigned long long gmask[NG];
     if (SPARSE) {
 #pragma unroll
-      for (int S = 0; S < 4; ++S) gmask[S] = __ballot(go && lo < 8 * S + 8 && hi > 8 * S);
+      for (int S = 0; S < NG; ++S) gmask[S] = __ballot(go && lo < 8 * S + 8 && hi > 8 * S);
     }
     if (!go) return;
-    auto group = [&](auto sidx, auto off, auto nbases) {
+    const uint32_t* const row_hi = s_kb + NW * (hi > KROWS - 1 ? KROWS - 1 : hi);
+    const uint32_t* const row_lo = s_kb + NW * (lo < 0 ? 0 : lo);
+    auto group = [&](auto sidx, auto nbases) {
       constexpr int S = decltype(sidx)::value;
       if (SPARSE && gmask[S] == 0ull) return;
       uint32_t x0 = bv[2 * S], x1 = bv[2 * S + 1];
       if (masked) {
-        const uint2 kh = *reinterpret_cast<const uint2*>(s_kb + 8 * (hi > 32 ? 32 : hi) + 2 * S);
-        const uint2 kl = *reinterpret_cast<const uint2*>(s_kb + 8 * (lo < 0 ? 0 : lo) + 2 * S);
+        const uint2 kh = *reinterpret_cast<const uint2*>(row_hi + 2 * S);
+        const uint2 kl = *reinterpret_cast<const uint2*>(row_lo + 2 * S);
         x0 &= kh.x & ~kl.x;
         x1 &= kh.y & ~kl.y;
       }
-      tally_group<decltype(off)::value, decltype(nbases)::value>(x0, x1, thr, abase, one);
+      tally_group<128 * S, decltype(nbases)::value>(x0, x1, thr, abase, one);
     };
     using std::integral_constant;
-    group(integral_constant<int, 0>{}, integral_constant<int, 0>{}, integral_constant<int, 8>{});
-    group(integral_constant<int, 1>{}, integral_constant<int, 128>{}, integral_constant<int, 8>{});
-    group(integral_constant<int, 2>{}, integral_constant<int, 256>{}, integral_constant<int, 8>{});
-    group(integral_constant<int, 3>{}, integral_constant<int, 384>{}, integral_constant<int, (LB == 32 ? 8 : 6)>{});
+    group(integral_constant<int, 0>{}, integral_constant<int, 8>{});
+    group(integral_constant<int, 1>{}, integral_constant<int, 8>{});
+    group(integral_constant<int, 2>{}, integral_constant<int, 8>{});
+    group(integral_constant<int, 3>{}, integral_constant<int, (NG > 4 ? 8 : LB - 24)>{});
+    if constexpr (NG > 4) group(integral_constant<int, 4>{}, integral_constant<int, LB - 32>{});
   };
 
   struct Raw { uint32_t pos, l_nc, nmq, off; };
@@ -236,7 +243,7 @@
     return f;
   };
   struct Rd { uint32_t pos, nmq, l_nc; };
-  struct Dat { uint32_t b[8]; uint32_t cg[4]; uint32_t qs; };
+  struct Dat { uint32_t b[NW]; uint32_t cg[4]; uint32_t qs; };
   auto settle = [&](const Raw& f, int n_reads_it, Rd& r, Dat& d) {
     const bool act = g < n_reads_it;
     const uint32_t l_nc = act ? f.l_nc : 0u;
@@ -257,6 +264,10 @@
     const uint32_t qs = *reinterpret_cast<const uint32_t*>(base + (size_t)vq);
     d.b[0] = ba.x; d.b[1] = ba.y; d.b[2] = ba.z; d.b[3] = ba.w;
     d.b[4] = bb.x; d.b[5] = bb.y; d.b[6] = bb.z; d.b[7] = bb.w;
+    if constexpr (NW > 8) {
+      const u32x2_a1 bc = *reinterpret_cast<const u32x2_a1*>(base + (size_t)vb + 32);
+      d.b[8] = bc.x; d.b[9] = bc.y;
+    }
     d.cg[0] = cv.x; d.cg[1] = cv.y; d.cg[2] = cv.z; d.cg[3] = cv.w;
     d.qs = qs;
   };
@@ -313,13 +324,13 @@
 #if MIDAS_SNPS_DEBUG_BITS & 256
       asm volatile("" :: "v"(rd_n.pos), "v"(rd_n.l_nc));
       const unsigned long long pt1 = PROBE_NOW();
-      asm volatile("" :: "v"(dat_cur.b[0]), "v"(dat_cur.b[7]), "v"(dat_cur.qs), "v"(dat_cur.cg[3]));
+      asm volatile("" :: "v"(dat_cur.b[0]), "v"(dat_cur.b[NW - 1]), "v"(dat_cur.qs), "v"(dat_cur.cg[3]));
       const unsigned long long pt2 = PROBE_NOW();
       pr_cols += pt1 - pt0; pr_bases += pt2 - pt1; pr_iters += 1;
 #endif
 
       if (kDebug & 4) {
-        asm volatile("" :: "v"(dat_cur.b[0]), "v"(dat_cur.b[7]), "v"(dat_cur.qs), "v"(dat_cur.cg[0]), "v"(rd_cur.pos));
+        asm volatile("" :: "v"(dat_cur.b[0]), "v"(dat_cur.b[NW - 1]), "v"(dat_cur.qs), "v"(dat_cur.cg[0]), "v"(rd_cur.pos));
         return;
       }
       MIDAS_MARK("qsum");
@@ -635,7 +646,11 @@
 
 int direct_lane_bases(int32_t max_l_seq) {
   const int l = max_l_seq > 0 ? max_l_seq : 1;
-  return (l + 31) / 32 < (l + 29) / 30 ? 32 : 30;
+  const int best = (l + 31) / 32 < (l + 29) / 30 ? 32 : 30;
+#ifndef MIDAS_DIRECT_NO_LB38
+  if (best == 30 && l > 96 && l <= kDirectOverhang && (l + 37) / 38 < (l + 31) / 32) return 38;
+#endif
+  return best;
 }
 
 hipError_t launch_pileup_direct(const DirectParams& p, int lane_bases, hipStream_t stream) {
@@ -645,6 +660,7 @@
   const int n_items = k > 1 ? p.n_chunked_tiles / k + (p.n_tiles - p.n_chunked_tiles) : p.n_tiles;
   const int grid = n_items < p.grid_blocks ? n_items : p.grid_blocks;
   const bool bq0 = p.baseq <= 0;
+  if (lane_bases != 30 && lane_bases != 32 && !(lane_bases == 38 && p.overhang <= kDirectOverhang)) return hipErrorInvalidValue;
   if (p.overhang > kDirectOverhang) {
     if (lane_bases == 32) {
       if (bq0) hipLaunchKernelGGL((pileup_direct_kernel<32, true, kDirectOverhangLong>), dim3(grid), dim3(kDirectBlock), dyn_lds, stream, p);
@@ -653,6 +669,9 @@
       if (bq0) hipLaunchKernelGGL((pileup_direct_kernel<30, true, kDirectOverhangLong>), dim3(grid), dim3(kDirectBlock), dyn_lds, stream, p);
       else hipLaunchKernelGGL((pileup_direct_kernel<30, false, kDirectOverhangLong>), dim3(grid), dim3(kDirectBlock), dyn_lds, stream, p);
     }
+  } else if (lane_bases == 38) {
+    if (bq0) hipLaunchKernelGGL((pileup_direct_kernel<38, true>), dim3(grid), dim3(kDirectBlock), dyn_lds, stream, p);
+    else hipLaunchKernelGGL((pileup_direct_kernel<38, false>), dim3(grid), dim3(kDirectBlock), dyn_lds, stream, p);
   } else if (lane_bases == 32) {
     if (bq0) hipLaunchKernelGGL((pileup_direct_kernel<32, true>), dim3(grid), dim3(kDirectBlock), dyn_lds, stream, p);
     else hipLaunchKernelGGL((pileup_direct_kernel<32, false>), dim3(grid), dim3(kDirectBlock), dyn_lds, stream, p);
```
